# regeirk/pycwt

Measured on NVIDIA H100. Metric: cwt_scale_points_per_sec, higher is better.
Workload: dtype f64

## Files before the change

profiles/micro/l2_bw.cu:

```cuda
#include <cstdio>
#include <cstdlib>
#include <cuda_runtime.h>

#define CK(x) do { cudaError_t e_ = (x); if (e_ != cudaSuccess) { printf("%s: %s\n", #x, cudaGetErrorString(e_)); exit(1); } } while (0)

__global__ void k_read(const double2 *__restrict__ a, size_t n, double2 *sink) {
  double2 acc = make_double2(0, 0);
  for (size_t i = (size_t)blockIdx.x * blockDim.x + threadIdx.x; i < n; i += (size_t)gridDim.x * blockDim.x) {
    double2 v = a[i];
    acc.x += v.x; acc.y += v.y;
  }
  if (acc.x == 1.2345e300) sink[0] = acc;
}
__global__ void k_write(double2 *__restrict__ a, size_t n, int streaming) {
  const double2 v = make_double2(1.0, 2.0);
  for (size_t i = (size_t)blockIdx.x * blockDim.x + threadIdx.x; i < n; i += (size_t)gridDim.x * blockDim.x) {
    if (streaming) __stcs(&a[i], v); else a[i] = v;
  }
}
__global__ void k_copy(const double2 *__restrict__ a, double2 *__restrict__ b, size_t n, int streaming) {
  for (size_t i = (size_t)blockIdx.x * blockDim.x + threadIdx.x; i < n; i += (size_t)gridDim.x * blockDim.x) {
    double2 v = a[i];
    if (streaming) __stcs(&b[i], v); else b[i] = v;
  }
}
__global__ void k_mix(const double2 *__restrict__ src, size_t nsrc, double2 *__restrict__ dst, size_t ndst) {
  for (size_t i = (size_t)blockIdx.x * blockDim.x + threadIdx.x; i < ndst; i += (size_t)gridDim.x * blockDim.x) {
    double2 v = src[i % nsrc];
    __stcs(&dst[i], v);
  }
}

template <class F> float timeit(F f, int reps) {
  cudaEvent_t e0, e1;
  CK(cudaEventCreate(&e0)); CK(cudaEventCreate(&e1));
  f();
  CK(cudaDeviceSynchronize());
  CK(cudaEventRecord(e0));
  for (int i = 0; i < reps; ++i) f();
  CK(cudaEventRecord(e1));
  CK(cudaEventSynchronize(e1));
  float ms = 0;
  CK(cudaEventElapsedTime(&ms, e0, e1));
  return ms / reps;
}

int main() {
  const size_t big = (size_t)1 << 30;
  double2 *A, *B, *sink;
  CK(cudaMalloc(&A, big)); CK(cudaMalloc(&B, big)); CK(cudaMalloc(&sink, 64));
  CK(cudaMemset(A, 1, big)); CK(cudaMemset(B, 1, big));
  const int grid = 132 * 8, block = 256;
  const size_t sizes_mb[] = {4, 8, 16, 24, 32, 48, 64, 96, 128, 256, 1024};
  printf("working set MB | read GB/s | write GB/s | write.cs GB/s | copy(r+w) GB/s | copy.cs GB/s\n");
  for (size_t mb : sizes_mb) {
    const size_t n = (mb << 20) / sizeof(double2);
    const int reps = mb <= 128 ? 50 : 10;
    const float tr = timeit([&] { k_read<<<grid, block>>>(A, n, sink); }, reps);
    const float tw = timeit([&] { k_write<<<grid, block>>>(A, n, 0); }, reps);
    const float tws = timeit([&] { k_write<<<grid, block>>>(A, n, 1); }, reps);
    const size_t nh = n / 2;
    const float tc = timeit([&] { k_copy<<<grid, block>>>(A, A + nh, nh, 0); }, reps);
    const float tcs = timeit([&] { k_copy<<<grid, block>>>(A, A + nh, nh, 1); }, reps);
    const double bytes = (double)n * sizeof(double2);
    printf("%6zu | %8.0f | %8.0f | %8.0f | %8.0f | %8.0f\n", mb, bytes / tr / 1e6, bytes / tw / 1e6,
           bytes / tws / 1e6, bytes / tc / 1e6, bytes / tcs / 1e6);
  }
  printf("mix: read an L2-resident source while streaming 1 GB of writes (GB/s counted on the WRITES)\n");
  const size_t src_mb[] = {8, 16, 32, 64, 1024};
  for (size_t mb : src_mb) {
    const size_t ns = (mb << 20) / sizeof(double2), nd = big / sizeof(double2);
    const float t = timeit([&] { k_mix<<<grid, block>>>(A, ns, B, nd); }, 10);
    printf("src %4zu MB: %8.0f GB/s written (+ the same read)\n", mb, (double)big / t / 1e6);
  }
  return 0;
}
```

pycwt_b200/csrc/engine.cu:

```cuda
#include <algorithm>
#include <array>
#include <cmath>
#include <cstdint>
#include <cstdio>
#include <cstdlib>
#include <cstring>
#include <map>
#include <mutex>
#include <set>
#include <string>
#include <type_traits>
#include <vector>

#include <cuda_runtime.h>
#ifndef CWTB_HOST_EMU
#include <dlfcn.h>
#endif

#include "../../include/cwt_b200.h"
#include "kernels.cuh"

using namespace cwtb;

template <class B, class = void> struct BodyNT { static constexpr int value = NT; };
template <class B> struct BodyNT<B, std::void_t<decltype(B::NTB)>> { static constexpr int value = B::NTB; };


#ifdef CWTB_HOST_EMU
typedef int rt_stream;
static inline int rt_malloc(void **p, size_t n) { *p = malloc(n ? n : 1); return *p ? 0 : 1; }
static inline int rt_free(void *p) { free(p); return 0; }
static inline int rt_host_alloc(void **p, size_t n) { *p = malloc(n ? n : 1); return *p ? 0 : 1; }
static inline int rt_host_free(void *p) { free(p); return 0; }
static inline int rt_h2d(void *d, const void *s, size_t n, rt_stream) { memcpy(d, s, n); return 0; }
static inline int rt_d2h(void *d, const void *s, size_t n, rt_stream) { memcpy(d, s, n); return 0; }
static inline int rt_memset(void *d, int v, size_t n, rt_stream) { memset(d, v, n); return 0; }
static inline int rt_sync(rt_stream) { return 0; }
static inline const char *rt_errstr(int) { return "emulation error"; }
#else
typedef cudaStream_t rt_stream;
static inline int rt_malloc(void **p, size_t n) { return (int)cudaMalloc(p, n ? n : 1); }
static inline int rt_free(void *p) { return (int)cudaFree(p); }
static inline int rt_host_alloc(void **p, size_t n) { return (int)cudaHostAlloc(p, n ? n : 1, cudaHostAllocDefault); }
static inline int rt_host_free(void *p) { return (int)cudaFreeHost(p); }
static inline int rt_h2d(void *d, const void *s, size_t n, rt_stream st) {
  return (int)cudaMemcpyAsync(d, s, n, cudaMemcpyHostToDevice, st);
}
static inline int rt_d2h(void *d, const void *s, size_t n, rt_stream st) {
  return (int)cudaMemcpyAsync(d, s, n, cudaMemcpyDeviceToHost, st);
}
static inline int rt_memset(void *d, int v, size_t n, rt_stream st) { return (int)cudaMemsetAsync(d, v, n, st); }
static inline int rt_sync(rt_stream st) { return (int)cudaStreamSynchronize(st); }
static inline const char *rt_errstr(int e) { return cudaGetErrorString((cudaError_t)e); }

template <class B, class = void> struct BodyMinB { static constexpr int value = CWTB_MINB; };
template <class B> struct BodyMinB<B, std::void_t<decltype(B::MINB)>> { static constexpr int value = B::MINB; };

template <class Body, int PH>
__device__ __forceinline__ void run_phases(const typename Body::Args &a, void *sm) {
  Body::template phase<PH>(a, (int)blockIdx.x, (int)blockIdx.y, (int)threadIdx.x, sm);
  if constexpr (PH + 1 < Body::NPHASE) {
    __syncthreads();
    run_phases<Body, PH + 1>(a, sm);
  }
}
template <class Body, int PH>
__device__ __forceinline__ void run_phases_at(const typename Body::Args &a, int bx, int by, void *sm) {
  Body::template phase<PH>(a, bx, by, (int)threadIdx.x, sm);
  if constexpr (PH + 1 < Body::NPHASE) {
    __syncthreads();
    run_phases_at<Body, PH + 1>(a, bx, by, sm);
  }
}
template <class Body>
__global__ void __launch_bounds__(BodyNT<Body>::value, BodyMinB<Body>::value) k_run(const __grid_constant__ typename Body::Args a) {
  extern __shared__ __align__(16) unsigned char smraw[];
  run_phases<Body, 0>(a, smraw);
}
#endif

struct Buf {
  void *p = nullptr;
  size_t bytes = 0;
};

struct ClassRun {
  int log2K;
  int first, count;
  int expand = 0;
  int log2Nc = 0;
  int taps = 0;
  long long woff = 0;
};

struct Job {
  bool valid = false;
  int precision = 0;
  long long n0 = 0;
  unsigned N = 0;
  int log2N = 0;
  int S = 0;
  int nbatch = 1;
  double dt = 0;
  Fam fam{};
  std::vector<ScaleDesc> descs;
  std::vector<ClassRun> classes;
  std::vector<int> plan_log2K;
  std::vector<double> scales;
  size_t b_single = 0;
  size_t coarse_elems = 0;
  int sig_is_f32 = 0;
  bool exact = false;
};

struct BluePlan {
  unsigned n = 0, L = 0;
  double2 *wm = nullptr;
  double2 *bf[2] = {nullptr, nullptr};
};

struct NTabDev {
  double2 *hi = nullptr, *lo = nullptr;
  int h = 0;
};

struct cwtb_ctx {
  int device = 0;
  rt_stream stream{};
  rt_stream aux_stream{};
  rt_stream prio_stream{};
  rt_stream prio_aux[7]{};
  int prio_fan = 4;
  int prio_mode = 1;
  rt_stream chain_streams[3]{};
  int n_chains = 2;
  rt_stream cur{};
  int pad_pow2 = 1;
  std::map<unsigned, BluePlan> blue;
  long long serial = 0;
  int two_streams = 1;
  int three_streams = 1;
  rt_stream copy_streams[4]{};
  int d2h_split = 1;
  std::string err;
  double band_eps = 1e-16;
  double band_eps32 = 1e-9;
  double expand_eps = 5e-13;
  double expand_eps32 = 2e-7;
  int expand_mma = 1;
  int dense_margin = 2;
  int expand_min_log2R = 3;
  Buf *ztmp = nullptr;
  void *comm = nullptr;
  int comm_world = 1, comm_rank = 0;
  Buf comm_send, comm_recv;
  int group = 0;
  size_t group_bytes = (size_t)512 << 20;
  size_t rows_chunk_bytes = (size_t)256 << 20;
  int l2_persist = 0;
  int direct_max_log2 = 13;
  int fused = 0;
  int ring = 3;
  int pipe_ahead = 2;
  int num_sms = 132;
  int pf_dist = 132;
  int gauss_rec = 1;
  int pf_rows_a = 32, pf_rows_b = 32;
  int pf_dist_a = 132;
  int k2_512_max_log2 = 16;
  int passb_rev = 1;
  int k2_band_log2 = 9;
  size_t batch_bytes = (size_t)4 << 30;
  double2 *tw64 = nullptr;
  float2 *tw32 = nullptr;
  std::map<unsigned, NTabDev> ntabs;
  Buf filt;
  int filt_rows = 0;
  long long filt_n = 0;
  Buf Zxs[7];
  Buf Zx, Cin, Cout, wtab;
  std::map<std::array<long long, 3>, long long> wtab_index;
  std::vector<double> wtab_host;
  size_t wtab_uploaded = 0;
  Buf ctr, sig, sig2, spec, Z, Zc[3], Y, B, W, W2, descs, table, scratch, C, A12, F, aux, rowd, win, mask, hist, noise, wide, blueA, blueX, blueY;
  Job job;
  struct PlanKey {
    long long n0 = -1;
    double dt = 0, param = 0, band_eps = 0, band_eps32 = 0, expand_eps = 0, expand_eps32 = 0;
    int S = 0, family = 0, precision = 0, nbatch = 0, pad = 0;
    std::vector<double> scales;
    bool operator==(const PlanKey &o) const {
      return n0 == o.n0 && dt == o.dt && param == o.param && band_eps == o.band_eps && band_eps32 == o.band_eps32 &&
             expand_eps == o.expand_eps && expand_eps32 == o.expand_eps32 && S == o.S && family == o.family &&
             precision == o.precision && nbatch == o.nbatch && pad == o.pad && scales == o.scales;
    }
  } plan_key;
  int plan_reuse = 1;
  void *stage_host[2] = {nullptr, nullptr};
  size_t stage_bytes = 0;
  Buf stage_dev[2], batch_power;
  int batch_pipeline = 1;
  double *angle_host = nullptr;
  const void *job_dsig = nullptr;
  double last_ms = 0;
  int launches = 0;
  std::set<const void *> configured;
  bool profiling = false;
  int prof_saved_streams = 1;
  const char *prof_tag = "";
  struct ProfRec { std::string name; unsigned gx, gy; int ev; };
  std::vector<ProfRec> prof;
#ifndef CWTB_HOST_EMU
  std::vector<cudaEvent_t> prof_events;
#endif
  std::set<void *> pinned, devallocs;
#ifndef CWTB_HOST_EMU
  cudaEvent_t e0{}, e1{};
  cudaEvent_t ev_fork{}, ev_join{}, ev_joinc[3]{}, ev_coarse{};
  cudaEvent_t ev_h2d[2]{}, ev_used[2]{};
  cudaEvent_t ev_xband{}, ev_pj[7]{}, ev_angle{};
#endif
};

static int fail(cwtb_ctx *c, int code, const std::string &msg);
static void apply_l2_policy(cwtb_ctx *c);
static int fail(cwtb_ctx *c, int code, const std::string &msg) {
  if (c) c->err = msg;
  return code;
}
#define RT(call)                                                                             \
  do {                                                                                       \
    int e_ = (call);                                                                         \
    if (e_ != 0) return fail(c, CWTB_ERR_CUDA, std::string(#call) + ": " + rt_errstr(e_));   \
  } while (0)
// ... 289 lines not shown
  fam.tpitch = N;
  double fconst = 1.0;
  if (family == CWTB_MORLET) fconst = std::pow(M_PI, -0.25);
  else if (family == CWTB_PAUL) {
    int m = (int)param;
    double fact = 1;
    for (int i = 2; i < 2 * m; ++i) fact *= i;
    fconst = std::pow(2.0, m) / std::sqrt(m * fact);
  } else if (family == CWTB_DOG) {
    int m = (int)param;
    fconst = 1.0 / std::sqrt(std::tgamma(m + 0.5));
    static const int unit_of[4] = {2, 1, 0, 3};
    fam.unit = unit_of[m & 3];
  }
  const double w1 = 6.283185307179586 * ((N == 2 ? -1.0 : 1.0) * fam.dw);
  double flo = 0, fhi = 0;
  bool pos_only = false;
  const double beps = (precision == CWTB_F32 && c->band_eps > 0) ? std::max(c->band_eps, c->band_eps32) : c->band_eps;
  if (family != CWTB_TABLE) family_band(family, param, beps, &flo, &fhi, &pos_only);

  std::vector<ScaleDesc> ds(S);
  job.plan_log2K.assign(S, 0);
  job.scales.assign(scales, scales + S);
  const long long half = (long long)N / 2;
  for (int j = 0; j < S; ++j) {
    ScaleDesc &d = ds[j];
    const double s = scales[j];
    d.s = s;
    d.row = j;
    d.trow = j;
    d.chan = 0;
    d.pad_ = 0;
    d.boff = 0;
    const double norm = std::sqrt(s * w1 * (double)N);
    d.amp = (family == CWTB_TABLE ? 1.0 : norm * fconst) / (double)N;
    long long klo = -half, khi = ((long long)N - 1) / 2;
    if (family != CWTB_TABLE && s > 0 && std::isfinite(s)) {
      const double cc = (double)N * dt / (6.283185307179586 * s);
      double a = std::ceil(flo * cc) - 1, b = std::floor(fhi * cc) + 1;
      if (a > (double)klo) klo = (long long)a;
      if (b < (double)khi) khi = (long long)b;
      if (pos_only && klo < 1) klo = 1;
    }
    if (N == 1) { klo = 0; khi = 0; }
    if (khi < klo) { klo = 1; khi = 0; }
    d.k_lo = (int)klo;
    d.k_hi = (int)khi;
    long long lo = std::min<long long>(klo, 0), hi = std::max<long long>(khi, 0);
    if (khi < klo) { lo = 0; hi = 0; }
    int lk = std::max(5, ilog2((unsigned long long)(hi - lo + 1)));
    if (lk > c->direct_max_log2) {
      lo = -((-lo + K2C - 1) / K2C) * K2C;
      lk = std::max(c->direct_max_log2 + 1, ilog2((unsigned long long)(hi - lo + 1)));
    }
    if (lk > 20) lk = job.log2N;
    const bool band_limited = lk < job.log2N;
    if (lk >= 18 && lk < job.log2N && job.log2N - lk <= c->dense_margin && job.log2N <= 20) lk = job.log2N;
    if (lk >= job.log2N) {
      lk = job.log2N;
      d.rsplit = (int)half;
      if (N == 1) d.rsplit = 1;
    } else {
      d.rsplit = (int)((1ll << lk) + lo);
    }
    d.log2K = lk;
    job.plan_log2K[j] = job.exact ? -1 : ((N < 32) ? 0 : lk);
    d.ip_log2Nc = 0; d.ip_kc = 0; d.ip_w = 0; d.ip_pad_ = 0; d.ip_coff = 0; d.ip_woff = 0;
    d.ip_beta = 0; d.ip_dc = 0;
    const double xeps = precision == CWTB_F64 ? c->expand_eps : c->expand_eps32;
    if (xeps > 0 && !job.exact && family != CWTB_TABLE && khi >= klo && job.log2N >= 9 && band_limited) {
      const long long kc = (klo + khi) / 2 - (((klo + khi) % 2 != 0 && (klo + khi) < 0) ? 1 : 0);
      const long long hw = std::max(khi - kc, kc - klo);
#ifdef CWTB_HOST_EMU
      const bool mma = false;
      const int max_taps = precision == CWTB_F64 ? 20 : 10;
#else
      const bool mma = precision == CWTB_F64 && c->expand_mma && job.log2N >= 12;
      const int max_taps = mma ? 20 : (precision == CWTB_F64 ? 16 : 10);
#endif
      const long long need = max_taps > 16 ? (32 * hw + 10) / 11 : 4 * hw;
      int lmin = std::max(6, ilog2((unsigned long long)std::max<long long>(need, 1)));
      lmin = std::max(lmin, job.log2N - 14);
      double best = 1e300;
      const int min_log2R = c->expand_min_log2R;
      for (int l = lmin; l <= lmin + 2 && job.log2N - l >= min_log2R; ++l) {
        double xi_b = 0;
        int w = expand_taps((double)hw / (double)(1ll << l), xeps, precision != CWTB_F64, max_taps, &xi_b);
        if (!w) continue;
        if (mma) w = (w + 3) / 4 * 4;
        if (xi_b > 0.25 && expand_gain(fam, s, klo, khi, kc, l, w, M_PI * w * (1.0 - xi_b)) > 64.0) continue;
        const int ksteps = job.log2N - l == 2 ? (w + 4) / 4 : (w + 3) / 4;
        const double xcost = mma ? std::max(2.72, 0.83 * ksteps) : 0.06 * (2 * w + 8);
        const double cost = xcost + (mma ? 18.0 : 12.0) * (double)(1ll << l) / (double)N;
        if (cost < best) {
          best = cost;
          d.ip_log2Nc = l; d.ip_kc = (int)kc; d.ip_w = w;
          d.ip_beta = M_PI * w * (1.0 - xi_b);
          d.ip_dc = std::cyl_bessel_i(0.0, d.ip_beta) / w;
        }
      }
      if (d.ip_log2Nc) {
        d.ip_woff = expand_weights(c, c->wtab_host, job.log2N - d.ip_log2Nc, d.ip_w, d.ip_beta);
        job.plan_log2K[j] = -d.ip_log2Nc;
      }
    }
  }
  if (nbatch > 1) {
    ds.resize((size_t)S * nbatch);
    for (int ch = 1; ch < nbatch; ++ch)
      for (int j = 0; j < S; ++j) {
        ScaleDesc d = ds[j];
        d.chan = ch;
        d.row = ch * S + j;
        ds[(size_t)ch * S + j] = d;
      }
  }
  const int R = S * nbatch;
  std::vector<int> order(R);
  for (int j = 0; j < R; ++j) order[j] = j;
  auto sort_key = [&](const ScaleDesc &d) -> long long {
    if (!d.ip_log2Nc) return (1ll << 40) + d.log2K;
    return ((long long)(64 - d.ip_w) << 32) + ((long long)d.ip_log2Nc << 24) - (d.ip_woff & 0xffffff);
  };
  std::stable_sort(order.begin(), order.end(), [&](int a, int b) { return sort_key(ds[a]) > sort_key(ds[b]); });
  job.descs.resize(R);
  size_t boff = 0, coff = 0;
  for (int i = 0; i < R; ++i) {
    job.descs[i] = ds[order[i]];
    ScaleDesc &d = job.descs[i];
    bool same = !job.classes.empty();
    if (same) {
      const ClassRun &b = job.classes.back();
      same = d.ip_log2Nc ? (b.expand && b.log2Nc == d.ip_log2Nc && b.taps == d.ip_w && b.woff == d.ip_woff)
                         : (!b.expand && b.log2K == d.log2K);
    }
    if (!same) {
      ClassRun cl{d.log2K, i, 0};
      if (d.ip_log2Nc) { cl.expand = 1; cl.log2Nc = d.ip_log2Nc; cl.taps = d.ip_w; cl.woff = d.ip_woff; }
      job.classes.push_back(cl);
    }
    job.classes.back().count++;
    if (d.ip_log2Nc) {
      d.ip_coff = (long long)coff;
      coff += (size_t)1 << d.ip_log2Nc;
    } else if (d.log2K <= 10 || (d.log2K <= c->direct_max_log2 && d.log2K < job.log2N)) {
      d.boff = (long long)boff;
      boff += (size_t)1 << d.log2K;
    }
  }
  job.b_single = boff;
  job.coarse_elems = coff;
  job.valid = true;
  return 0;
}

template <typename T> struct Tw;
template <> struct Tw<double> { static const double2 *get(cwtb_ctx *c) { return c->tw64; } };
template <> struct Tw<float> { static const float2 *get(cwtb_ctx *c) { return c->tw32; } };

template <typename T, int SIGN>
static int fft_rows(cwtb_ctx *c, const void *in, int real_in, long long in_pitch, long long n_in,
                    cx<T> *out, long long out_pitch, unsigned n, int nrows, long long nout = -1,
                    const double *grow = nullptr, double post = 1.0);

template <typename T, int SIGN, int K>
static int fft_rows_small(cwtb_ctx *c, const RowsArgs<T> &a) {
  constexpr int P = Lay<T, K>::P;
// ... 446 lines not shown
    RT(cudaFuncSetAttribute(kern, cudaFuncAttributeMaxDynamicSharedMemorySize, (int)smem));
    c->configured.insert(fn);
  }
  int occ = 0;
  RT(cudaOccupancyMaxActiveBlocksPerMultiprocessor(&occ, kern, TileCfg<T>::NT, smem));
  if (occ < 1) return fail(c, CWTB_ERR_CUDA, "pipelined kernel does not fit on an SM");
  const unsigned total = (unsigned)nscales * (f.tilesA + f.tilesB);
  const unsigned grid = std::min<unsigned>(total, (unsigned)(occ * c->num_sms));
  int ev = -1;
  if (c->profiling) {
    ev = (int)c->prof.size() * 2;
    while ((int)c->prof_events.size() < ev + 2) {
      cudaEvent_t e2;
      RT(cudaEventCreate(&e2));
      c->prof_events.push_back(e2);
    }
    char nm[64];
    snprintf(nm, sizeof nm, "PipeAB<%s, %d, %d>", sizeof(T) == 8 ? "double" : "float", K1, MODE);
    c->prof.push_back({nm, grid, (unsigned)nscales, ev});
    RT(cudaEventRecord(c->prof_events[ev], c->cur));
  }
  kern<<<grid, TileCfg<T>::NT, smem, c->cur>>>(f);
  RT(cudaGetLastError());
  if (ev >= 0) RT(cudaEventRecord(c->prof_events[ev + 1], c->cur));
  c->launches++;
  return 0;
#endif
}

template <typename T, int MODE>
static int dispatch_pipe(cwtb_ctx *c, int log2K1, const PassAArgs<T> &a, const PassBArgs<T> &b, int n) {
  switch (log2K1) {
    case 4: return launch_pipe<T, 16, MODE>(c, a, b, n);
    case 5: return launch_pipe<T, 32, MODE>(c, a, b, n);
    case 6: return launch_pipe<T, 64, MODE>(c, a, b, n);
    case 7: return launch_pipe<T, 128, MODE>(c, a, b, n);
    case 8: return launch_pipe<T, 256, MODE>(c, a, b, n);
    case 9: return launch_pipe<T, 512, MODE>(c, a, b, n);
    case 10: return launch_pipe<T, 1024, MODE>(c, a, b, n);
  }
  return fail(c, CWTB_ERR_UNSUPPORTED, "pipelined two-pass kernel: unsupported first-pass length");
}

template <typename T, int K>
static int launch_single(cwtb_ctx *c, const SingleArgs<T> &a, int count) {
  constexpr int P = Lay<T, K>::P;
  const unsigned M = a.N / K;
  return launch<SingleBody<T, K>>(c, (M + P - 1) / P, count, a);
}

static int chunk_rows(const cwtb_ctx *c, unsigned N, size_t elem_bytes) {
  if (c->group > 0) return c->group;
  size_t g = c->group_bytes / ((size_t)N * elem_bytes);
  return (int)std::max<size_t>(1, std::min<size_t>(g, 32768));
}

static bool class_single(const cwtb_ctx *c, const Job &job, const ClassRun &cl) {
  return !cl.expand && (cl.log2K <= 10 || (cl.log2K <= c->direct_max_log2 && cl.log2K < job.log2N));
}
static bool class_two_kernel(const cwtb_ctx *c, const Job &job, const ClassRun &cl) {
  return !cl.expand && !class_single(c, job, cl);
}
static bool class_persistent(const cwtb_ctx *c, const ClassRun &cl) {
  return c->fused == 1 || (c->fused == 2 && cl.log2K >= 14 && cl.log2K <= 20 && cl.count <= 256);
}

static int job_chain_region(const cwtb_ctx *c, const Job &job, const ClassRun &cl) {
  int idx = 0;
  for (const ClassRun &o : job.classes) {
    if (&o == &cl) break;
    if (class_two_kernel(c, job, o)) ++idx;
  }
  return idx % std::max(1, c->n_chains);
}

static size_t band_chunk_elems(const cwtb_ctx *c, const Job &job, int G) {
  size_t bchunk = 0;
  for (const ClassRun &cl : job.classes)
    if (class_two_kernel(c, job, cl) && cl.log2K < job.log2N)
      bchunk = std::max(bchunk, (size_t)(class_persistent(c, cl) ? cl.count : std::min(G, cl.count)) << cl.log2K);
  return bchunk;
}

template <typename T, int TAPS>
static int launch_expand_t(cwtb_ctx *c, const ExpandArgs<T> &a, int rows, int min_log2Nc) {
  using B = ExpandBody<T, TAPS>;
  const unsigned gx = std::max<unsigned>(1, a.N / (unsigned)(B::NT * B::L));
#ifndef CWTB_HOST_EMU
  if constexpr (std::is_same<T, double>::value) {
    static_assert(ExpandMmaBody<TAPS>::OUT_PER_CTA == 4096, "the planner assumes the tensor-core kernel from Np = 2^12");
    if (c->expand_mma && a.N >= (unsigned)ExpandMmaBody<TAPS>::OUT_PER_CTA) {
      const unsigned gm = a.N / (32u * std::min<unsigned>(ExpandMmaBody<TAPS>::L, 1u << min_log2Nc));
      if (a.epi == EPI_MULCONJ) return launch<ExpandMmaBody<TAPS, EPI_MULCONJ>>(c, gm, rows, a);
      return launch<ExpandMmaBody<TAPS>>(c, gm, rows, a);
    }
  }
#endif
#ifndef CWTB_HOST_EMU
  if constexpr (TAPS > 16) {
    return fail(c, CWTB_ERR_STATE, "expansion: tap counts above 16 exist on the tensor-core kernel only");
  } else
#endif
  {
    if (a.epi == EPI_MULCONJ) return launch<ExpandBody<T, TAPS, EPI_MULCONJ>>(c, gx, rows, a);
    return launch<B>(c, gx, rows, a);
  }
}
template <typename T>
static int launch_expand(cwtb_ctx *c, int taps, const ExpandArgs<T> &a, int rows, int min_log2Nc) {
  if constexpr (std::is_same<T, double>::value) {
    switch (taps) {
      case 10: return launch_expand_t<T, 10>(c, a, rows, min_log2Nc);
      case 12: return launch_expand_t<T, 12>(c, a, rows, min_log2Nc);
      case 14: return launch_expand_t<T, 14>(c, a, rows, min_log2Nc);
      case 16: return launch_expand_t<T, 16>(c, a, rows, min_log2Nc);
      case 20: return launch_expand_t<T, 20>(c, a, rows, min_log2Nc);
    }
  } else {
    switch (taps) {
      case 6: return launch_expand_t<T, 6>(c, a, rows, min_log2Nc);
      case 8: return launch_expand_t<T, 8>(c, a, rows, min_log2Nc);
      case 10: return launch_expand_t<T, 10>(c, a, rows, min_log2Nc);
    }
  }
  return fail(c, CWTB_ERR_STATE, "expansion: unsupported tap count");
}

template <typename T>
static int run_job(cwtb_ctx *c, const Job &job, const T *dsig, cx<T> *Wout = nullptr, int epi = EPI_STORE) {
  using V = cx<T>;
  if (job.exact) {
    if constexpr (std::is_same<T, double>::value) return run_job_exact(c, job, dsig, Wout, epi);
    else return fail(c, CWTB_ERR_UNSUPPORTED, "un-padded transforms run in fp64");
  }
  const unsigned N = job.N;
  const int S = job.S * job.nbatch;
  int e;
  struct CurGuard { cwtb_ctx *c; ~CurGuard() { c->cur = c->stream; c->prof_tag = ""; c->ztmp = nullptr; } } cur_guard{c};
  if ((e = ensure(c, c->spec, (size_t)job.nbatch * N * sizeof(V)))) return e;
  if (!Wout) {
    if ((e = ensure(c, c->W, (size_t)S * job.n0 * sizeof(V)))) return e;
    Wout = (V *)c->W.p;
  }
  V *spec = (V *)c->spec.p;
  V *W = Wout;
  const ScaleDesc *ddesc = (const ScaleDesc *)c->descs.p;
  Fam fam = job.fam;
  if (fam.family == CWTB_TABLE) fam.table = (const double2 *)c->table.p;

  if (N < 32) {
    if (job.nbatch != 1) return fail(c, CWTB_ERR_UNSUPPORTED, "batched transform needs n0 > 16");
    TinyFwdArgs<T> fa{dsig, spec, job.n0, N};
    if ((e = launch<TinyFwdBody<T>>(c, 1, 1, fa))) return e;
    TinyArgs<T> ta{ddesc, spec, W, fam, job.n0, N, 0, epi};
    return launch<TinyBody<T>>(c, (unsigned)((job.n0 + NT - 1) / NT), S, ta);
  }
  c->prof_tag = "fwd:";
  e = fft_rows<T, -1>(c, dsig, 1, job.n0, job.n0, spec, N, N, job.nbatch);
  c->prof_tag = "";
  if (e) return e;

  NTab nt;
  if ((e = get_ntab(c, N, job.log2N, &nt))) return e;
  const int G = chunk_rows(c, N, sizeof(V));
  const size_t bchunk = band_chunk_elems(c, job, G);
  if ((e = ensure(c, c->B, (job.b_single + (size_t)std::max(1, c->n_chains) * bchunk) * sizeof(V)))) return e;
  V *Bbuf = (V *)c->B.p;

  {
    int first = -1, maxlk = 0, nrows = 0;
    for (const ClassRun &cl : job.classes)
      if (class_single(c, job, cl)) {
        if (first < 0) first = cl.first;
        maxlk = std::max(maxlk, cl.log2K);
        nrows += cl.count;
      }
    if (first >= 0) {
// ... 1573 lines not shown
```

pycwt_b200/csrc/kernels.cuh:

```cuda
#pragma once
#include <math.h>
#include "fft_tile.cuh"

namespace cwtb {

struct ScaleDesc {
  double s;
  double amp;
  int row;
  int k_lo, k_hi;
  int log2K;
  int rsplit;
  int trow;
  int chan;
  int pad_;
  long long boff;
  int ip_log2Nc;
  int ip_kc;
  int ip_w;
  int ip_pad_;
  long long ip_coff;
  long long ip_woff;
  double ip_beta;
  double ip_dc;
// ... 681 lines not shown
    const int R = 1 << log2R;
    const int Nc = 1 << d.ip_log2Nc;
    const int RB = R < NT ? R : NT;
    const int NRUN = NT / RB;
    const int MT = NRUN * L;
    const int mtiles = (Nc + MT - 1) / MT;
    const int mt = bx % mtiles, rb = bx / mtiles;
    if (rb * RB >= R) return;
    const int m0 = mt * MT;
    if constexpr (PH == 0) {
      const V *c = a.C + d.ip_coff;
      for (int i = tid; i < MT + TAPS; i += NT) {
        const int m = (m0 - (TAPS / 2 - 1) + i) & (Nc - 1);
        sm[skew(i)] = ldg(&c[m]);
      }
    } else {
      const int rl = tid & (RB - 1), j = tid / RB;
      const int rho = rb * RB + rl;
      const int ms = m0 + j * L;
      const long long nfirst = ((long long)ms << log2R) + rho;
      long long keep = (a.n0 - nfirst + R - 1) >> log2R;
      if (keep > Nc - ms) keep = Nc - ms;
      const int smax = keep < 0 ? 0 : (keep > L ? L : (int)keep);
      if (smax == 0) return;
      T hw[TAPS];
      const double *wt = a.wt + d.ip_woff + rho;
#pragma unroll
      for (int t = 0; t < TAPS; ++t) hw[t] = (T)ldg(&wt[(size_t)t * R]);
      const V *run = sm + 33 * j;
      V win[TAPS];
#pragma unroll
      for (int t = 0; t < TAPS - 1; ++t) win[t] = run[t + (t >> 5)];
      constexpr int RESEED = sizeof(T) == 8 ? 16 : 8;
      const unsigned kc = (unsigned)d.ip_kc;
      const unsigned nlo = (unsigned)nfirst;
      const V stepw = nroot_t<T>(a.nt, kc << log2R);
      V tw = mk<T>(1, 0);
      V *p = a.W + (size_t)d.row * a.n0 + nfirst;
#pragma unroll
      for (int s = 0; s < L; ++s) {
        win[(s + TAPS - 1) % TAPS] = run[(s + TAPS - 1) + ((s + TAPS - 1) >> 5)];
        if (s % RESEED == 0) tw = nroot_t<T>(a.nt, kc * (nlo + ((unsigned)s << log2R)));
        constexpr int NCH = sizeof(T) == 8 ? 4 : 2;
        T ar[4] = {0, 0, 0, 0}, ai[4] = {0, 0, 0, 0};
#pragma unroll
        for (int t = 0; t < TAPS; ++t) {
          const V cv = win[(s + t) % TAPS];
          ar[t & (NCH - 1)] += cv.x * hw[t];
          ai[t & (NCH - 1)] += cv.y * hw[t];
        }
        const V acc = NCH == 4 ? mk<T>((ar[0] + ar[1]) + (ar[2] + ar[3]), (ai[0] + ai[1]) + (ai[2] + ai[3]))
                               : mk<T>(ar[0] + ar[1], ai[0] + ai[1]);
        const V x = cmul(acc, tw);
        tw = cmul(tw, stepw);
        if (s < smax) {
          if (EPI == EPI_MULCONJ) *p = cmul(*p, cconj(x));
          else st_stream(p, x);
        }
        p += R;
      }
    }
  }
};

#ifndef CWTB_HOST_EMU
__device__ __forceinline__ void dmma884(double &c0, double &c1, double a, double b) {
  asm volatile("mma.sync.aligned.m8n8k4.row.col.f64.f64.f64.f64 {%0,%1}, {%2}, {%3}, {%0,%1};"
               : "+d"(c0), "+d"(c1) : "d"(a), "d"(b));
}
template <int TAPS, int EPI = EPI_STORE> struct ExpandMmaBody {
  static constexpr int NTB = 128;
  static constexpr int NT = NTB;
  static constexpr int MINB = 4;
  using V = double2;
  using Args = ExpandArgs<double>;
#ifndef CWTB_MMA_L
#define CWTB_MMA_L 128
#endif
  static constexpr int L = CWTB_MMA_L;
  static constexpr int KS = (TAPS + 3) / 4;
  static constexpr int KS4 = (TAPS + 4) / 4;
  static constexpr int OUT_PER_CTA = 32 * L;
  static constexpr int STAGE = 8 * L + 4 * KS4;
  static constexpr int NPHASE = 2;
  static constexpr size_t SMEM = (size_t)STAGE * sizeof(V);
  template <int PH> __device__ static void phase(const Args &a, int bx, int by, int tid, void *smraw) {
    const ScaleDesc &d = a.descs[a.first + by];
    if (a.log2N - d.ip_log2Nc == 2) body<PH, true>(a, d, bx, tid, (V *)smraw);
    else body<PH, false>(a, d, bx, tid, (V *)smraw);
  }
  template <int PH, bool R4>
  __device__ static void body(const Args &a, const ScaleDesc &d, int bx, int tid, V *sm) {
    constexpr int KSr = R4 ? KS4 : KS;
    constexpr int Lr = R4 ? 2 * L : L;
    constexpr int MB = R4 ? 16 : 8;
    const int log2R = a.log2N - d.ip_log2Nc;
    const int R = 1 << log2R;
    const int Nc = 1 << d.ip_log2Nc;
    const int wpb = R4 ? 1 : ((R < 32 ? R : 32) >> 3);
    const int nrun = 4 / wpb;
    const int MT = nrun * Lr;
    const int mtiles = (Nc + MT - 1) / MT;
    const int mt = bx % mtiles, rb = bx / mtiles;
    if (rb * 32 >= R && rb > 0) return;
    const int m0 = mt * MT;
    if constexpr (PH == 0) {
      const V *c = a.C + d.ip_coff;
      for (int i = tid; i < MT + 4 * KSr; i += NT) sm[i] = ldg(&c[(m0 - (TAPS / 2 - 1) + i) & (Nc - 1)]);
    } else {
      const int wid = tid >> 5, lane = tid & 31;
      const int g = lane >> 2, q = lane & 3;
      const int pb = wid % wpb, j = wid / wpb;
      const int rho0 = R4 ? 0 : rb * 32 + pb * 8;
      const int ms = m0 + j * Lr;
      double bf[KSr];
#pragma unroll
      for (int ks = 0; ks < KSr; ++ks) {
        const int t = 4 * ks + q - (R4 ? (g >> 2) : 0);
        const int rho = R4 ? (g & 3) : rho0 + g;
        bf[ks] = (t >= 0 && t < TAPS) ? ldg(&a.wt[d.ip_woff + (size_t)t * R + rho]) : 0.0;
      }
      const unsigned kc = (unsigned)d.ip_kc;
      const int mlane = R4 ? 2 * g + (q >> 1) : g;
      const int rlane = R4 ? 2 * (q & 1) : rho0 + 2 * q;
      const unsigned n00 = ((unsigned)(ms + mlane) << log2R) + (unsigned)rlane;
      V tw0 = nroot(a.nt, kc * n00);
      V tw1 = cmul(tw0, nroot(a.nt, kc));
      const V stepb = nroot(a.nt, (kc * (unsigned)MB) << log2R);
      const V *run = sm + j * Lr + (R4 ? 2 * g : g) + q;
      V *rowp = a.W + (size_t)d.row * a.n0;
#pragma unroll 4
      for (int mb = 0; mb < Lr / MB; ++mb) {
        if (ms + MB * mb >= Nc) break;
        double cr0 = 0, cr1 = 0, ci0 = 0, ci1 = 0;
#pragma unroll
        for (int ks = 0; ks < KSr; ++ks) {
          const V s = run[MB * mb + 4 * ks];
          dmma884(cr0, cr1, s.x, bf[ks]);
          dmma884(ci0, ci1, s.y, bf[ks]);
        }
        const int m = ms + MB * mb + mlane;
        const long long n = ((long long)m << log2R) + rlane;
        V x0 = cmul(make_double2(cr0, ci0), tw0);
        V x1 = cmul(make_double2(cr1, ci1), tw1);
        tw0 = cmul(tw0, stepb);
        tw1 = cmul(tw1, stepb);
        if (m < Nc && n < a.n0) {
          V *p = rowp + n;
          const bool two = n + 1 < a.n0;
          if (EPI == EPI_MULCONJ) {
            x0 = cmul(p[0], cconj(x0));
            if (two) x1 = cmul(p[1], cconj(x1));
            p[0] = x0;
            if (two) p[1] = x1;
          } else {
            st_stream(p, x0);
            if (two) st_stream(p + 1, x1);
          }
        }
      }
    }
  }
};
#endif

template <typename T> struct BandArgs {
  const ScaleDesc *descs;
  const cx<T> *spec;
  cx<T> *Bbuf;
  Fam fam;
  unsigned N;
  int first;
};
template <typename T> struct BandBody {
  using V = cx<T>;
  using Args = BandArgs<T>;
  static constexpr int NPHASE = 1;
  static constexpr size_t SMEM = 0;
  static constexpr int PER = 4;
  template <int PH> HD static void phase(const Args &a, int bx, int by, int tid, void *) {
    const ScaleDesc d = a.descs[a.first + by];
    const int K = 1 << d.log2K;
#pragma unroll
    for (int i = 0; i < PER; ++i) {
      const int r = (bx * PER + i) * NT + tid;
      if (r >= K) return;
      const int k = r - (r >= d.rsplit ? K : 0);
      V v = mk<T>(0, 0);
      if (k >= d.k_lo && k <= d.k_hi) v = band_value<T>(a.fam, d, a.spec, (unsigned)k & (a.N - 1), k, a.N);
      a.Bbuf[d.boff + r] = v;
    }
  }
};

template <typename T> struct RowsArgs {
  const void *in;
  cx<T> *out;
  const cx<T> *tw;
  const double *grow;
  long long in_pitch, out_pitch, n_in, nout;
  double post;
  int nrows, real_in, n;
};

template <typename T, int K> struct RowsLoader {
  using V = cx<T>;
  const RowsArgs<T> *a;
  int row0;
  int base, stride;
  HD void begin(int base_, int stride_, int, int) { base = base_; stride = stride_; }
  HD V get(int b, int pos) const {
    const int row = row0 + b;
    if (row >= a->nrows || pos >= a->n_in) return mk<T>(0, 0);
    if (a->real_in) return mk<T>(ldg((const T *)a->in + (size_t)row * a->in_pitch + pos), (T)0);
    return ldg((const V *)a->in + (size_t)row * a->in_pitch + pos);
  }
  template <int R> HD void load(int b, V (&x)[R]) const {
#pragma unroll
    for (int i = 0; i < R; ++i) x[i] = get(b, base + i * stride);
  }
};
template <typename T> struct RowsStorer {
  using V = cx<T>;
  const RowsArgs<T> *a;
  int row0;
  template <int R> HD void store(int b, int ql, int qs, V (&x)[R]) const {
    const int row = row0 + b;
    if (row >= a->nrows) return;
#pragma unroll
    for (int c = 0; c < R; ++c) {
      const int q = ql + c * qs;
      if (q >= a->nout) continue;
      V v = x[c];
      if (a->grow) {
        Epilogue<T> e;
        e.mode = EPI_GAUSS; e.g = a->grow[row]; e.invn = 1.0 / (double)a->n; e.post = a->post; e.nfreq = a->n;
        v = e.apply(v, v, q);
      }
      a->out[(size_t)row * a->out_pitch + q] = v;
    }
// ... 637 lines not shown
```

Baseline: 89.96 billion.

## Make tensor-core expand kernel persistent with cp.async double buffering and shuffle-coalesced stores

```diff
diff --git a/profiles/micro/l2_bw.cu b/profiles/micro/l2_bw.cu
--- a/profiles/micro/l2_bw.cu
+++ b/profiles/micro/l2_bw.cu
@@ -29,6 +29,50 @@
     double2 v = src[i % nsrc];
     __stcs(&dst[i], v);
   }
+}
+
+__global__ void k_write_pair16(double2 *__restrict__ a, size_t nchunk, int xchg) {
+  const int lane = threadIdx.x & 31;
+  const size_t w0 = ((size_t)blockIdx.x * blockDim.x + threadIdx.x) >> 5, nw = ((size_t)gridDim.x * blockDim.x) >> 5;
+  const double2 v = make_double2(1.0, 2.0);
+  for (size_t c = w0; c < nchunk; c += nw) {
+    double2 *p = a + c * 64 + 2 * lane;
+    if (xchg) {
+      const int odd = lane & 1;
+      __stcs(p - odd, v);
+      __stcs(p + 2 - odd, v);
+    } else {
+      __stcs(p, v);
+      __stcs(p + 1, v);
+    }
+  }
+}
+template <int RUN> __global__ void k_write_bulk(double2 *__restrict__ a, size_t nchunk) {
+  __shared__ __align__(128) double2 ring[4][4][64];
+  const int lane = threadIdx.x & 31, wid = threadIdx.x >> 5;
+  const size_t w0 = ((size_t)blockIdx.x * blockDim.x + threadIdx.x) >> 5, nw = ((size_t)gridDim.x * blockDim.x) >> 5;
+  unsigned long long pol;
+  asm volatile("createpolicy.fractional.L2::evict_first.b64 %0, 1.0;" : "=l"(pol));
+  int slot = 0;
+  for (size_t c = w0; c < nchunk; c += nw) {
+    if (lane == 0) asm volatile("cp.async.bulk.wait_group.read 3;" ::: "memory");
+    __syncwarp();
+    double2 *s = ring[wid][slot];
+    s[2 * lane] = make_double2(1.0, 2.0);
+    s[2 * lane + 1] = make_double2(1.0, 2.0);
+    asm volatile("fence.proxy.async.shared::cta;" ::: "memory");
+    __syncwarp();
+    if (lane == 0) {
+      for (int r = 0; r < 1024 / RUN; ++r) {
+        const unsigned sa = (unsigned)__cvta_generic_to_shared((char *)s + r * RUN);
+        asm volatile("cp.async.bulk.global.shared::cta.bulk_group.L2::cache_hint [%0], [%1], %2, %3;"
+                     ::"l"((char *)(a + c * 64) + r * RUN), "r"(sa), "n"(RUN), "l"(pol) : "memory");
+      }
+      asm volatile("cp.async.bulk.commit_group;" ::: "memory");
+    }
+    slot = (slot + 1) & 3;
+  }
+  if (lane == 0) asm volatile("cp.async.bulk.wait_group 0;" ::: "memory");
 }
 
 template <class F> float timeit(F f, int reps) {
@@ -73,5 +117,25 @@
     const float t = timeit([&] { k_mix<<<grid, block>>>(A, ns, B, nd); }, 10);
     printf("src %4zu MB: %8.0f GB/s written (+ the same read)\n", mb, (double)big / t / 1e6);
   }
+  CK(cudaFree(A)); CK(cudaFree(B));
+  const size_t huge = (size_t)4 << 30, nchunk = huge / 1024;
+  double2 *H;
+  CK(cudaMalloc(&H, huge));
+  CK(cudaMemset(H, 1, huge));
+  const size_t nh = huge / sizeof(double2);
+  const int g128 = 132 * 16;
+  printf("write patterns, 4 GiB buffer (GB/s):\n");
+  for (int rep = 0; rep < 3; ++rep) {
+    const float ta = timeit([&] { k_write<<<g128, 128>>>(H, nh, 1); }, 5);
+    const float tb = timeit([&] { k_write_pair16<<<g128, 128>>>(H, nchunk, 0); }, 5);
+    const float td = timeit([&] { k_write_pair16<<<g128, 128>>>(H, nchunk, 1); }, 5);
+    const float tc1 = timeit([&] { k_write_bulk<1024><<<g128, 128>>>(H, nchunk); }, 5);
+    const float tc2 = timeit([&] { k_write_bulk<128><<<g128, 128>>>(H, nchunk); }, 5);
+    CK(cudaGetLastError());
+    printf("  (a) coalesced st.cs %6.0f | (b) pair16 st.cs %6.0f | (b') pair16 exchanged %6.0f | "
+           "(c) bulk 1 KiB %6.0f | (c) bulk 128 B %6.0f\n", huge / ta / 1e6, huge / tb / 1e6, huge / td / 1e6,
+           huge / tc1 / 1e6, huge / tc2 / 1e6);
+  }
+  CK(cudaFree(H));
   return 0;
 }
diff --git a/pycwt_b200/csrc/engine.cu b/pycwt_b200/csrc/engine.cu
--- a/pycwt_b200/csrc/engine.cu
+++ b/pycwt_b200/csrc/engine.cu
@@ -76,6 +76,12 @@
 __global__ void __launch_bounds__(BodyNT<Body>::value, BodyMinB<Body>::value) k_run(const __grid_constant__ typename Body::Args a) {
   extern __shared__ __align__(16) unsigned char smraw[];
   run_phases<Body, 0>(a, smraw);
+}
+template <class Body>
+__global__ void __launch_bounds__(Body::NTB, Body::MINB) k_persist(const __grid_constant__ typename Body::Args a,
+                                                                   unsigned gm, unsigned total) {
+  extern __shared__ __align__(16) unsigned char smraw[];
+  Body::run_tiles(a, gm, total, (typename Body::V *)smraw);
 }
 #endif
 
@@ -149,7 +155,7 @@
   double expand_eps32 = 2e-7;
   int expand_mma = 1;
   int dense_margin = 2;
-  int expand_min_log2R = 3;
+  int expand_min_log2R = 0;
   Buf *ztmp = nullptr;
   void *comm = nullptr;
   int comm_world = 1, comm_rank = 0;
@@ -605,7 +611,7 @@
       int lmin = std::max(6, ilog2((unsigned long long)std::max<long long>(need, 1)));
       lmin = std::max(lmin, job.log2N - 14);
       double best = 1e300;
-      const int min_log2R = c->expand_min_log2R;
+      const int min_log2R = c->expand_min_log2R ? c->expand_min_log2R : (mma ? 2 : 3);
       for (int l = lmin; l <= lmin + 2 && job.log2N - l >= min_log2R; ++l) {
         double xi_b = 0;
         int w = expand_taps((double)hw / (double)(1ll << l), xeps, precision != CWTB_F64, max_taps, &xi_b);
@@ -1218,6 +1224,41 @@
   return bchunk;
 }
 
+#ifndef CWTB_HOST_EMU
+template <class Body>
+static int launch_persistent(cwtb_ctx *c, unsigned gm, unsigned rows, const typename Body::Args &a) {
+  if (gm == 0 || rows == 0) return 0;
+  auto kern = k_persist<Body>;
+  const void *fn = (const void *)kern;
+  if (!c->configured.count(fn)) {
+    RT(cudaFuncSetAttribute(kern, cudaFuncAttributeMaxDynamicSharedMemorySize, (int)Body::SMEM));
+    c->configured.insert(fn);
+  }
+  int occ = 0;
+  RT(cudaOccupancyMaxActiveBlocksPerMultiprocessor(&occ, kern, Body::NTB, Body::SMEM));
+  if (occ < 1) return fail(c, CWTB_ERR_CUDA, "persistent kernel does not fit on an SM");
+  const unsigned long long total = (unsigned long long)gm * rows;
+  if (total > 0xffffffffull) return fail(c, CWTB_ERR_ARG, "too many tiles in one launch");
+  const unsigned grid = (unsigned)std::min<unsigned long long>(total, (unsigned long long)occ * c->num_sms);
+  int ev = -1;
+  if (c->profiling) {
+    ev = (int)c->prof.size() * 2;
+    while ((int)c->prof_events.size() < ev + 2) {
+      cudaEvent_t e;
+      RT(cudaEventCreate(&e));
+      c->prof_events.push_back(e);
+    }
+    c->prof.push_back({std::string(c->prof_tag) + body_name(__PRETTY_FUNCTION__), grid, rows, ev});
+    RT(cudaEventRecord(c->prof_events[ev], c->cur));
+  }
+  kern<<<grid, Body::NTB, Body::SMEM, c->cur>>>(a, gm, (unsigned)total);
+  RT(cudaGetLastError());
+  if (ev >= 0) RT(cudaEventRecord(c->prof_events[ev + 1], c->cur));
+  c->launches++;
+  return 0;
+}
+#endif
+
 template <typename T, int TAPS>
 static int launch_expand_t(cwtb_ctx *c, const ExpandArgs<T> &a, int rows, int min_log2Nc) {
   using B = ExpandBody<T, TAPS>;
@@ -1227,8 +1268,8 @@
     static_assert(ExpandMmaBody<TAPS>::OUT_PER_CTA == 4096, "the planner assumes the tensor-core kernel from Np = 2^12");
     if (c->expand_mma && a.N >= (unsigned)ExpandMmaBody<TAPS>::OUT_PER_CTA) {
       const unsigned gm = a.N / (32u * std::min<unsigned>(ExpandMmaBody<TAPS>::L, 1u << min_log2Nc));
-      if (a.epi == EPI_MULCONJ) return launch<ExpandMmaBody<TAPS, EPI_MULCONJ>>(c, gm, rows, a);
-      return launch<ExpandMmaBody<TAPS>>(c, gm, rows, a);
+      if (a.epi == EPI_MULCONJ) return launch_persistent<ExpandMmaBody<TAPS, EPI_MULCONJ>>(c, gm, rows, a);
+      return launch_persistent<ExpandMmaBody<TAPS>>(c, gm, rows, a);
     }
   }
 #endif
diff --git a/pycwt_b200/csrc/kernels.cuh b/pycwt_b200/csrc/kernels.cuh
--- a/pycwt_b200/csrc/kernels.cuh
+++ b/pycwt_b200/csrc/kernels.cuh
@@ -787,32 +787,66 @@
   static constexpr int KS4 = (TAPS + 4) / 4;
   static constexpr int OUT_PER_CTA = 32 * L;
   static constexpr int STAGE = 8 * L + 4 * KS4;
-  static constexpr int NPHASE = 2;
-  static constexpr size_t SMEM = (size_t)STAGE * sizeof(V);
-  template <int PH> __device__ static void phase(const Args &a, int bx, int by, int tid, void *smraw) {
-    const ScaleDesc &d = a.descs[a.first + by];
-    if (a.log2N - d.ip_log2Nc == 2) body<PH, true>(a, d, bx, tid, (V *)smraw);
-    else body<PH, false>(a, d, bx, tid, (V *)smraw);
-  }
-  template <int PH, bool R4>
-  __device__ static void body(const Args &a, const ScaleDesc &d, int bx, int tid, V *sm) {
+  static constexpr size_t SMEM = 2 * (size_t)STAGE * sizeof(V);
+  struct Tile {
+    const ScaleDesc *d;
+    int log2R, Nc, wpb, MT, m0, rb;
+    bool r4, live;
+  };
+  __device__ static Tile tile(const Args &a, unsigned w, unsigned gm) {
+    Tile t;
+    const int bx = (int)(w % gm);
+    t.d = &a.descs[a.first + (int)(w / gm)];
+    t.log2R = a.log2N - t.d->ip_log2Nc;
+    t.r4 = t.log2R == 2;
+    const int R = 1 << t.log2R;
+    t.Nc = 1 << t.d->ip_log2Nc;
+    t.wpb = t.r4 ? 1 : ((R < 32 ? R : 32) >> 3);
+    t.MT = (4 / t.wpb) * (t.r4 ? 2 * L : L);
+    const int mtiles = (t.Nc + t.MT - 1) / t.MT;
+    t.rb = bx / mtiles;
+    t.m0 = (bx % mtiles) * t.MT;
+    t.live = !(t.rb * 32 >= R && t.rb > 0);
+    return t;
+  }
+  __device__ static void load(const Args &a, const Tile &t, V *sm) {
+    if (!t.live) return;
+    const V *c = a.C + t.d->ip_coff;
+    const int n = t.MT + 4 * (t.r4 ? KS4 : KS);
+    for (int i = (int)threadIdx.x; i < n; i += NT) cp_async(&sm[i], &c[(t.m0 - (TAPS / 2 - 1) + i) & (t.Nc - 1)]);
+  }
+  __device__ static void run_tiles(const Args &a, unsigned gm, unsigned total, V *sm) {
+    unsigned w = blockIdx.x;
+    Tile cur = tile(a, w, gm);
+    load(a, cur, sm);
+    for (int st = 0; w < total; w += gridDim.x, st ^= 1) {
+      cp_async_wait();
+      __syncthreads();
+      const unsigned wn = w + gridDim.x;
+      Tile nxt = cur;
+      if (wn < total) {
+        nxt = tile(a, wn, gm);
+        load(a, nxt, sm + (st ^ 1) * STAGE);
+      }
+      if (cur.live) {
+        if (cur.r4) compute<true>(a, cur, sm + st * STAGE);
+        else compute<false>(a, cur, sm + st * STAGE);
+      }
+      cur = nxt;
+    }
+  }
+  template <bool R4>
+  __device__ static void compute(const Args &a, const Tile &tl, const V *sm) {
     constexpr int KSr = R4 ? KS4 : KS;
     constexpr int Lr = R4 ? 2 * L : L;
     constexpr int MB = R4 ? 16 : 8;
-    const int log2R = a.log2N - d.ip_log2Nc;
+    const ScaleDesc &d = *tl.d;
+    const int log2R = tl.log2R;
     const int R = 1 << log2R;
-    const int Nc = 1 << d.ip_log2Nc;
-    const int wpb = R4 ? 1 : ((R < 32 ? R : 32) >> 3);
-    const int nrun = 4 / wpb;
-    const int MT = nrun * Lr;
-    const int mtiles = (Nc + MT - 1) / MT;
-    const int mt = bx % mtiles, rb = bx / mtiles;
-    if (rb * 32 >= R && rb > 0) return;
-    const int m0 = mt * MT;
-    if constexpr (PH == 0) {
-      const V *c = a.C + d.ip_coff;
-      for (int i = tid; i < MT + 4 * KSr; i += NT) sm[i] = ldg(&c[(m0 - (TAPS / 2 - 1) + i) & (Nc - 1)]);
-    } else {
+    const int Nc = tl.Nc;
+    const int wpb = tl.wpb, rb = tl.rb, m0 = tl.m0;
+    {
+      const int tid = (int)threadIdx.x;
       const int wid = tid >> 5, lane = tid & 31;
       const int g = lane >> 2, q = lane & 3;
       const int pb = wid % wpb, j = wid / wpb;
@@ -846,21 +880,25 @@
         }
         const int m = ms + MB * mb + mlane;
         const long long n = ((long long)m << log2R) + rlane;
-        V x0 = cmul(make_double2(cr0, ci0), tw0);
-        V x1 = cmul(make_double2(cr1, ci1), tw1);
+        const V x0 = cmul(make_double2(cr0, ci0), tw0);
+        const V x1 = cmul(make_double2(cr1, ci1), tw1);
         tw0 = cmul(tw0, stepb);
         tw1 = cmul(tw1, stepb);
-        if (m < Nc && n < a.n0) {
-          V *p = rowp + n;
-          const bool two = n + 1 < a.n0;
+        const bool odd = q & 1;
+        const V snd = odd ? x0 : x1;
+        const V rcv = make_double2(__shfl_xor_sync(0xffffffffu, snd.x, 1), __shfl_xor_sync(0xffffffffu, snd.y, 1));
+        const long long na = odd ? n - 1 : n;
+        V ya = odd ? rcv : x0;
+        V yb = odd ? x1 : rcv;
+        if (m < Nc) {
+          V *p = rowp + na;
+          const bool sa = na < a.n0, sb = na + 2 < a.n0;
           if (EPI == EPI_MULCONJ) {
-            x0 = cmul(p[0], cconj(x0));
-            if (two) x1 = cmul(p[1], cconj(x1));
-            p[0] = x0;
-            if (two) p[1] = x1;
+            if (sa) p[0] = cmul(p[0], cconj(ya));
+            if (sb) p[2] = cmul(p[2], cconj(yb));
           } else {
-            st_stream(p, x0);
-            if (two) st_stream(p + 1, x1);
+            if (sa) st_stream(p, ya);
+            if (sb) st_stream(p + 2, yb);
           }
         }
       }
```

Measured after the change: 96.11 billion (median of 6 runs). 1.07x the previous value.
